# Tencent/PocketFlow

Measured on AMD Instinct MI355X. Metric: images/sec ResNet-50 INT8 quant-aware fine-tune (whole job; per GPU = value / n_gpus), higher is better.
Workload: dtype bf16

## Files before the change

### pocketflow_amd/csrc/pf_wrw.hip

```cpp
#include "pf_conv_common.h"
#include <stdlib.h>

#define LDS_PTR(p) ((__attribute__((address_space(3))) void*)(p))
typedef short v4s __attribute__((ext_vector_type(4)));
typedef short v8s __attribute__((ext_vector_type(8)));

__device__ __attribute__((aligned(16))) const uint32_t pf_wrw_zero_page[64] = {0};

struct WrwArgs {
  const bf16_t* dY;
  const bf16_t* X;
  float* slabs;
  const float* ss;
  const uint32_t* slot;
  float kq, act_lo, act_hi;
  int M, N, C;
  int th, tw, H, Wd, Ho, Wo, stride, pad_h, pad_w;
  int tiles_n, tiles, rows_per_split;
};

template <int N> __device__ __forceinline__ void wrw_wait_vm() { asm volatile("s_waitcnt vmcnt(%0)" ::"n"(N) : "memory"); }

template <int BN, bool PRO, bool MAP>
__global__ __launch_bounds__(256) void k_wrw_tr(const WrwArgs a) {
  constexpr int NB = BN / 16;
  constexpr int NS = 3;
  constexpr int DY_BYTES = 4 * NB * 256, X_BYTES = 4 * 4 * 256, STAGE = DY_BYTES + X_BYTES;
  constexpr int LPS = NB + 4;
  constexpr int NBLK = NB * 4;
  extern __shared__ __attribute__((aligned(16))) unsigned char smem[];
  const int tid = threadIdx.x, lane = tid & 63;
  const int wave = __builtin_amdgcn_readfirstlane(tid >> 6);
  const int l15 = lane & 15, q = lane >> 4;
  unsigned char* ring = smem + wave * (NS * STAGE);
  const bf16_t* zero = reinterpret_cast<const bf16_t*>(pf_wrw_zero_page);

  const int nwg = gridDim.x;
  int wg = blockIdx.x;
  {
    const int xcd = wg & 7, idx = wg >> 3;
    const int qq = nwg >> 3, r = nwg & 7;
    wg = (xcd < r ? xcd * (qq + 1) : r * (qq + 1) + (xcd - r) * qq) + idx;
  }
  const int tile = wg % a.tiles, split = wg / a.tiles;
  const int tn = tile % a.tiles_n, tk = tile / a.tiles_n;
  const int n0 = tn * BN;
  const int cch = a.C >> 6;
  const int tap = tk / cch, c0 = (tk - tap * cch) * 64;
  const int tap_r = tap / a.tw, tap_s = tap - tap_r * a.tw;
  const int ktot = a.th * a.tw * a.C;
  const int mbeg = split * a.rows_per_split;
  const int mend = (mbeg + a.rows_per_split < a.M) ? (mbeg + a.rows_per_split) : a.M;
  const int nsteps = (mend > mbeg) ? (mend - mbeg + 31) / 32 : 0;
  const int my_steps = (nsteps > wave) ? (nsteps - wave + 3) / 4 : 0;

  float psc[4], psh[4];
  Pro pro;
  pro_init(pro, a.act_lo, a.act_hi, a.kq, PRO ? a.slot : nullptr);
  if (PRO) {
#pragma unroll
    for (int j = 0; j < 4; ++j) {
      psc[j] = pro_fold_scale(pro, a.ss[c0 + j * 16 + l15]);
      psh[j] = pro_fold_shift(pro, a.ss[a.C + c0 + j * 16 + l15]);
    }
  }

  const int sb = lane >> 4, srow = (lane & 15) >> 1, sch = lane & 1;
  const int hw_o = a.Ho * a.Wo;
  auto stage = [&](int step, int buf) {
    unsigned char* dst = ring + buf * STAGE;
    const int mb = mbeg + step * 32;
#pragma unroll
    for (int pg = 0; pg < 4; ++pg) {
      const int m = mb + pg * 8 + srow;
      const bool ok = m < mend;
#pragma unroll
      for (int g4 = 0; g4 < NB / 4; ++g4) {
        const int n = n0 + (g4 * 4 + sb) * 16 + sch * 8;
        const bf16_t* src = (ok && n < a.N) ? (a.dY + (int64_t)m * a.N + n) : (zero + sch * 8);
        __builtin_amdgcn_global_load_lds(src, LDS_PTR(dst + (pg * NB + g4 * 4) * 256), 16, 0, 0);
      }
      bool okx = ok;
      int64_t row = m;
      if (MAP && ok) {
        const int img = m / hw_o, rem = m - img * hw_o;
        const int ho = rem / a.Wo, wo = rem - ho * a.Wo;
        const int hi = ho * a.stride + tap_r - a.pad_h, wi = wo * a.stride + tap_s - a.pad_w;
        okx = (unsigned)hi < (unsigned)a.H && (unsigned)wi < (unsigned)a.Wd;
        row = ((int64_t)img * a.H + hi) * a.Wd + wi;
      }
      const bf16_t* srcx = okx ? (a.X + row * a.C + c0 + sb * 16 + sch * 8) : (zero + sch * 8);
      __builtin_amdgcn_global_load_lds(srcx, LDS_PTR(dst + DY_BYTES + pg * 4 * 256), 16, 0, 0);
    }
  };

  f32x4 acc[NB][4];
#pragma unroll
  for (int i = 0; i < NB; ++i)
#pragma unroll
    for (int j = 0; j < 4; ++j) acc[i][j] = (f32x4){0.f, 0.f, 0.f, 0.f};

  const int tr_off = (q & 1) * 128 + (l15 >> 2) * 32 + (l15 & 3) * 8;
  const int pg_lo = q >> 1;

  if (my_steps > 0) stage(wave, 0);
  if (my_steps > 1) stage(wave + 4, 1);
  int ibuf = 2, cbuf = 0;
  for (int t = 0; t < my_steps; ++t) {
    if (t + 2 < my_steps) {
      stage(wave + (t + 2) * 4, ibuf);
      ibuf = (ibuf == NS - 1) ? 0 : ibuf + 1;
      wrw_wait_vm<2 * LPS>();
    } else if (t + 1 < my_steps) {
      wrw_wait_vm<LPS>();
    } else {
      wrw_wait_vm<0>();
    }
    __builtin_amdgcn_sched_barrier(0);
    const unsigned char* sbase = ring + cbuf * STAGE;
    cbuf = (cbuf == NS - 1) ? 0 : cbuf + 1;
    bf16x8 xf[4];
#pragma unroll
    for (int j = 0; j < 4; ++j) {
      const v4s lo = __builtin_amdgcn_ds_read_tr16_b64_v4i16(
          (__attribute__((address_space(3))) v4s*)(sbase + DY_BYTES + (pg_lo * 4 + j) * 256 + tr_off));
      const v4s hi = __builtin_amdgcn_ds_read_tr16_b64_v4i16(
          (__attribute__((address_space(3))) v4s*)(sbase + DY_BYTES + ((pg_lo + 2) * 4 + j) * 256 + tr_off));
      uint4 u;
      u.x = (uint32_t)(uint16_t)lo[0] | ((uint32_t)(uint16_t)lo[1] << 16);
      u.y = (uint32_t)(uint16_t)lo[2] | ((uint32_t)(uint16_t)lo[3] << 16);
      u.z = (uint32_t)(uint16_t)hi[0] | ((uint32_t)(uint16_t)hi[1] << 16);
      u.w = (uint32_t)(uint16_t)hi[2] | ((uint32_t)(uint16_t)hi[3] << 16);
      if (PRO) {
        float f[8];
        unpack8(u, f);
#pragma unroll
        for (int e = 0; e < 8; ++e) f[e] = pro_point(pro, psc[j], psh[j], f[e]);
        u = pack8(f);
      }
      xf[j] = *reinterpret_cast<const bf16x8*>(&u);
    }
#pragma unroll
    for (int i = 0; i < NB; ++i) {
      const v4s lo = __builtin_amdgcn_ds_read_tr16_b64_v4i16(
          (__attribute__((address_space(3))) v4s*)(sbase + (pg_lo * NB + i) * 256 + tr_off));
      const v4s hi = __builtin_amdgcn_ds_read_tr16_b64_v4i16(
          (__attribute__((address_space(3))) v4s*)(sbase + ((pg_lo + 2) * NB + i) * 256 + tr_off));
      v8s d8;
      d8[0] = lo[0]; d8[1] = lo[1]; d8[2] = lo[2]; d8[3] = lo[3];
      d8[4] = hi[0]; d8[5] = hi[1]; d8[6] = hi[2]; d8[7] = hi[3];
      const bf16x8 df = *reinterpret_cast<const bf16x8*>(&d8);
#pragma unroll
      for (int j = 0; j < 4; ++j)
        acc[i][j] = __builtin_amdgcn_mfma_f32_16x16x32_bf16(df, xf[j], acc[i][j], 0, 0, 0);
    }
  }

  __syncthreads();
  float4* red = reinterpret_cast<float4*>(smem);
#pragma unroll
  for (int i = 0; i < NB; ++i)
#pragma unroll
    for (int j = 0; j < 4; ++j)
      red[(wave * NBLK + i * 4 + j) * 64 + lane] = make_float4(acc[i][j][0], acc[i][j][1], acc[i][j][2], acc[i][j][3]);
  __syncthreads();
  float* out = a.slabs + (int64_t)split * a.N * ktot;
  const int kcol = tap * a.C + c0;
#pragma unroll
  for (int b = 0; b < NBLK / 4; ++b) {
    const int blk = wave * (NBLK / 4) + b;
    const int i = blk >> 2, j = blk & 3;
    float4 s = red[(0 * NBLK + blk) * 64 + lane];
#pragma unroll
    for (int w = 1; w < 4; ++w) {
      const float4 v = red[(w * NBLK + blk) * 64 + lane];
      s.x += v.x; s.y += v.y; s.z += v.z; s.w += v.w;
    }
    const int k = kcol + j * 16 + l15;
    const int n = n0 + i * 16 + q * 4;
    const float e[4] = {s.x, s.y, s.z, s.w};
#pragma unroll
    for (int r = 0; r < 4; ++r)
      if (n + r < a.N) out[(int64_t)(n + r) * ktot + k] = e[r];
  }
}

static bool wrw_tr_1x1_enabled() {
  return pf_tuning().wrw_tr != 0;
}

int pf_wrw_tr_splits(int M, int N, int C, int taps);
int pf_wrw2_splits(int M, int N, int C, int taps);
int pf_wrw_tr_splits_1x1(int M, int N, int C) {
  const int s2 = pf_wrw2_splits(M, N, C, 1);
  if (s2 > 0) return s2;
  return wrw_tr_1x1_enabled() ? pf_wrw_tr_splits(M, N, C, 1) : 0;
}

static int wrw_tr_bn(int N) { return (N % 128 == 0) ? 128 : 64; }

int pf_wrw_tr_splits(int M, int N, int C, int taps) {
  if ((C % 64) || (N % 64) || M < 2048) return 0;
  const int bn = wrw_tr_bn(N);
  const int tiles = (N / bn) * (taps * C / 64);
  int S = (256 + tiles - 1) / tiles;
  const int maxS = (M + 511) / 512;
  if (S > maxS) S = maxS;
  if (S < 1) S = 1;
  int rows = (M + S - 1) / S;
  rows = ((rows + 127) / 128) * 128;
  return (M + rows - 1) / rows;
}

template <int BN, bool PRO, bool MAP>
static int wrw_tr_launch_t(const WrwArgs& a, int grid, hipStream_t st) {
  constexpr int NB = BN / 16;
  const size_t ring = 4 * (size_t)3 * ((4 * NB + 16) * 256);
  const size_t red = (size_t)4 * NB * 4 * 64 * 16;
  const size_t lds = ring > red ? ring : red;
  if (int e = pf_require_lds(reinterpret_cast<const void*>(&k_wrw_tr<BN, PRO, MAP>), lds)) return e;
  k_wrw_tr<BN, PRO, MAP><<<grid, 256, lds, st>>>(a);
  PF_LAUNCH_CHECK();
  return 0;
}

int pf_wrw_tr_launch(const void* dY, const void* X, float* slabs, const float* scale_shift, int act,
                     const uint32_t* slot, int bits, int M, int N, int C, int th, int tw, int H, int Wd, int Ho, int Wo,
                     int stride, int pad_h, int pad_w, int S, hipStream_t st) {
  if (S <= 0) return -1;
  WrwArgs a;
  a.dY = (const bf16_t*)dY; a.X = (const bf16_t*)X; a.slabs = slabs;
  a.ss = scale_shift; a.slot = slot;
  a.kq = uq_k_of_bits(slot ? bits : 8);
  a.act_lo = (act == PF_ACT_NONE) ? -INFINITY : 0.0f;
  a.act_hi = (act == PF_ACT_RELU6) ? 6.0f : INFINITY;
  a.M = M; a.N = N; a.C = C; a.th = th; a.tw = tw; a.H = H; a.Wd = Wd; a.Ho = Ho; a.Wo = Wo;
  a.stride = stride; a.pad_h = pad_h; a.pad_w = pad_w;
  const int bn = wrw_tr_bn(N);
  a.tiles_n = N / bn;
  a.tiles = a.tiles_n * (th * tw * C / 64);
  int rows = (M + S - 1) / S;
  rows = ((rows + 127) / 128) * 128;
  a.rows_per_split = rows;
  const int grid = a.tiles * S;
  const bool pro = scale_shift != nullptr;
  const bool map = stride != 1 || th * tw > 1;
  if (pro && th * tw > 1) return -1;
#define PF_WT(BNV)                                                                            \
  do {                                                                                        \
    if (pro) return map ? wrw_tr_launch_t<BNV, true, true>(a, grid, st) : wrw_tr_launch_t<BNV, true, false>(a, grid, st);   \
    return map ? wrw_tr_launch_t<BNV, false, true>(a, grid, st) : wrw_tr_launch_t<BNV, false, false>(a, grid, st);          \
  } while (0)
  if (bn == 128) PF_WT(128);
  PF_WT(64);
#undef PF_WT
}

#if defined(__HIP_DEVICE_COMPILE__)
typedef __amdgpu_buffer_rsrc_t pf_wrsrc_t;
#define PF_W_MAKE_RSRC(p, bytes) __builtin_amdgcn_make_buffer_rsrc((void*)(p), (short)0, (int)(bytes), 0x00020000)
#define PF_W_BUFFER_LOAD_LDS16(rs, lds, voff) __builtin_amdgcn_raw_ptr_buffer_load_lds(rs, LDS_PTR(lds), 16, voff, 0, 0, 0)
#else
typedef int pf_wrsrc_t;
#define PF_W_MAKE_RSRC(p, bytes) 0
#define PF_W_BUFFER_LOAD_LDS16(rs, lds, voff) ((void)(rs), (void)(lds), (void)(voff))
#endif

#ifndef PF_W2_ABLATE
#define PF_W2_ABLATE 0
#endif
#ifdef PF_W2_TIMING
#define PF_W2_STAMP(k) do { if (blockIdx.x == (unsigned)tm_blk && t >= 4 && t < 12 && lane == 0) \
    tm_out[(t - 4) * 8 + (k)] = (uint32_t)__builtin_readcyclecounter(); } while (0)
#else
#define PF_W2_STAMP(k) do { } while (0)
#endif

__device__ __forceinline__ bf16x8 tr_join(const v4s& lo, const v4s& hi) {
  v8s x8;
  x8[0] = lo[0]; x8[1] = lo[1]; x8[2] = lo[2]; x8[3] = lo[3];
  x8[4] = hi[0]; x8[5] = hi[1]; x8[6] = hi[2]; x8[7] = hi[3];
  return *reinterpret_cast<const bf16x8*>(&x8);
}
template <int HI>
__device__ __forceinline__ void tr_read_frags(uint32_t p, bf16x8 (&f)[4]) {
  v4s l0, l1, l2, l3, h0, h1, h2, h3;
  asm volatile("ds_read_b64_tr_b16 %0, %8\n\tds_read_b64_tr_b16 %4, %8 offset:%9\n\t"
               "ds_read_b64_tr_b16 %1, %8 offset:256\n\tds_read_b64_tr_b16 %5, %8 offset:%10\n\t"
               "ds_read_b64_tr_b16 %2, %8 offset:512\n\tds_read_b64_tr_b16 %6, %8 offset:%11\n\t"
               "ds_read_b64_tr_b16 %3, %8 offset:768\n\tds_read_b64_tr_b16 %7, %8 offset:%12\n\t"
               "s_waitcnt lgkmcnt(0)"
               : "=&v"(l0), "=&v"(l1), "=&v"(l2), "=&v"(l3), "=&v"(h0), "=&v"(h1), "=&v"(h2), "=&v"(h3)
               : "v"(p), "n"(HI), "n"(HI + 256), "n"(HI + 512), "n"(HI + 768)
               : "memory");
  f[0] = tr_join(l0, h0); f[1] = tr_join(l1, h1); f[2] = tr_join(l2, h2); f[3] = tr_join(l3, h3);
}
template <int HI>
__device__ __forceinline__ void tr_read_frags(uint32_t p, bf16x8 (&f)[2]) {
  v4s l0, l1, h0, h1;
  asm volatile("ds_read_b64_tr_b16 %0, %4\n\tds_read_b64_tr_b16 %2, %4 offset:%5\n\t"
               "ds_read_b64_tr_b16 %1, %4 offset:256\n\tds_read_b64_tr_b16 %3, %4 offset:%6\n\t"
               "s_waitcnt lgkmcnt(0)"
               : "=&v"(l0), "=&v"(l1), "=&v"(h0), "=&v"(h1)
               : "v"(p), "n"(HI), "n"(HI + 256)
               : "memory");
  f[0] = tr_join(l0, h0); f[1] = tr_join(l1, h1);
}

template <int HIX, int HID>
__device__ __forceinline__ void tr_read_frags2(uint32_t px, uint32_t pd, bf16x8 (&xf)[4], bf16x8 (&df)[4]) {
  v4s a0, a1, a2, a3, b0, b1, b2, b3, c0, c1, c2, c3, d0, d1, d2, d3;
  asm volatile("ds_read_b64_tr_b16 %0, %16\n\tds_read_b64_tr_b16 %4, %16 offset:%18\n\t"
               "ds_read_b64_tr_b16 %1, %16 offset:256\n\tds_read_b64_tr_b16 %5, %16 offset:%19\n\t"
               "ds_read_b64_tr_b16 %2, %16 offset:512\n\tds_read_b64_tr_b16 %6, %16 offset:%20\n\t"
               "ds_read_b64_tr_b16 %3, %16 offset:768\n\tds_read_b64_tr_b16 %7, %16 offset:%21\n\t"
               "ds_read_b64_tr_b16 %8, %17\n\tds_read_b64_tr_b16 %12, %17 offset:%22\n\t"
               "ds_read_b64_tr_b16 %9, %17 offset:256\n\tds_read_b64_tr_b16 %13, %17 offset:%23\n\t"
               "ds_read_b64_tr_b16 %10, %17 offset:512\n\tds_read_b64_tr_b16 %14, %17 offset:%24\n\t"
               "ds_read_b64_tr_b16 %11, %17 offset:768\n\tds_read_b64_tr_b16 %15, %17 offset:%25\n\t"
               "s_waitcnt lgkmcnt(0)"
               : "=&v"(a0), "=&v"(a1), "=&v"(a2), "=&v"(a3), "=&v"(b0), "=&v"(b1), "=&v"(b2), "=&v"(b3),
                 "=&v"(c0), "=&v"(c1), "=&v"(c2), "=&v"(c3), "=&v"(d0), "=&v"(d1), "=&v"(d2), "=&v"(d3)
               : "v"(px), "v"(pd), "n"(HIX), "n"(HIX + 256), "n"(HIX + 512), "n"(HIX + 768), "n"(HID), "n"(HID + 256), "n"(HID + 512),
                 "n"(HID + 768)
               : "memory");
  xf[0] = tr_join(a0, b0); xf[1] = tr_join(a1, b1); xf[2] = tr_join(a2, b2); xf[3] = tr_join(a3, b3);
  df[0] = tr_join(c0, d0); df[1] = tr_join(c1, d1); df[2] = tr_join(c2, d2); df[3] = tr_join(c3, d3);
}

struct Wrw2Args {
  const bf16_t* dY;
  const bf16_t* X;
  float* slabs;
  const float* ss;
  const uint32_t* slot;
  float kq, act_lo, act_hi;
  uint32_t dy_bytes, x_bytes;
  int M, N, C;
  int th, tw, H, Wd, Ho, Wo, stride, pad_h, pad_w;
  int tiles_n, tiles, rows_per_split;
};

template <int TN, int TK, int WTN, int WTK, bool PRO, int MAPM>
__global__ __launch_bounds__(64 * (TN / WTN) * (TK / WTK)) void k_wrw2(const Wrw2Args a) {
  constexpr int WN = TN / WTN, WK = TK / WTK, NWAVE = WN * WK;
  constexpr int NI = WTN / 16, NJ = WTK / 16;
  constexpr int NBN = TN / 16, NBK = TK / 16;
  constexpr int DY_BYTES = 4 * NBN * 256, X_BYTES = 4 * NBK * 256, STAGE = DY_BYTES + X_BYTES;
  constexpr int IDY = 4 * (TN / 64), IX = 4 * (TK / 64);
  static_assert(IDY % NWAVE == 0 || IDY < NWAVE, "dY instructions must split evenly over the wavefronts (slot kinds are static)");
  constexpr int KDY = (IDY + NWAVE - 1) / NWAVE;
  constexpr int XS = (IX + NWAVE - 1) / NWAVE;
  extern __shared__ __attribute__((aligned(16))) unsigned char smem[];
  const int tid = threadIdx.x, lane = tid & 63;
  const int wave = __builtin_amdgcn_readfirstlane(tid >> 6);
  const int l15 = lane & 15, q = lane >> 4;
  const int wn = wave / WK, wk = wave % WK;

  const int nwg = gridDim.x;
  int wg = blockIdx.x;
  {
    const int xcd = wg & 7, idx = wg >> 3;
    const int qq = nwg >> 3, r = nwg & 7;
    wg = (xcd < r ? xcd * (qq + 1) : r * (qq + 1) + (xcd - r) * qq) + idx;
  }
  const int tile = wg % a.tiles, split = wg / a.tiles;
  const int tn = tile % a.tiles_n, tk = tile / a.tiles_n;
  const int n0 = tn * TN;
  const int kt = a.C / TK;
  const int tap = tk / kt, c0 = (tk - tap * kt) * TK;
  const int tap_r = tap / a.tw, tap_s = tap - tap_r * a.tw;
  const int ktot = a.th * a.tw * a.C;
  const int mbeg = split * a.rows_per_split;
  const int mend = (mbeg + a.rows_per_split < a.M) ? (mbeg + a.rows_per_split) : a.M;
  const int nsteps = (mend > mbeg) ? (mend - mbeg + 31) / 32 : 0;

  const pf_wrsrc_t rsY = PF_W_MAKE_RSRC(a.dY, (uint32_t)mend * (uint32_t)a.N * 2u);
  const pf_wrsrc_t rsX = PF_W_MAKE_RSRC(a.X, (MAPM == 0) ? (uint32_t)mend * (uint32_t)a.C * 2u : a.x_bytes);
  constexpr uint32_t OOB = 0x80000000u;
  const int sb = lane >> 4, srow = (lane & 15) >> 1, sch = lane & 1;
  const int hw_o = a.Ho * a.Wo;

  float psc[XS][8], psh[XS][8];
  Pro pro;
  pro_init(pro, a.act_lo, a.act_hi, a.kq, PRO ? a.slot : nullptr);
  if (PRO) {
#pragma unroll
    for (int x = 0; x < XS; ++x) {
      const int xi = wave + x * NWAVE;
      if (xi < IX) {
        const int g4 = xi % (TK / 64);
        const int c = c0 + (g4 * 4 + sb) * 16 + sch * 8;
#pragma unroll
        for (int j = 0; j < 8; ++j) { psc[x][j] = pro_fold_scale(pro, a.ss[c + j]); psh[x][j] = pro_fold_shift(pro, a.ss[a.C + c + j]); }
      }
    }
  }

  uint32_t yoff[KDY], xoff[XS];
  const uint32_t ystep = 32u * (uint32_t)a.N * 2u, xstep = 32u * (uint32_t)a.C * 2u;
#pragma unroll
  for (int k = 0; k < KDY; ++k) {
    const int id = (wave + k * NWAVE) % IDY;
    const int pg = id / (TN / 64), g4 = id % (TN / 64);
    const int n = n0 + (g4 * 4 + sb) * 16 + sch * 8;
    yoff[k] = (n < a.N && wave + k * NWAVE < IDY) ? (uint32_t)((mbeg + pg * 8 + srow) * a.N + n) * 2u : OOB;
  }
  int px_img[XS], px_ho[XS], px_wo[XS];
  const int adv_q = 32 / a.Wo, adv_r = 32 - adv_q * a.Wo;
  const int tap_dr = tap_r - a.pad_h, tap_ds = tap_s - a.pad_w;
#pragma unroll
  for (int x = 0; x < XS; ++x) {
    const int xi = (wave + x * NWAVE) % IX;
    const int pg = xi / (TK / 64), g4 = xi % (TK / 64);
    const int m = mbeg + pg * 8 + srow;
    const int cofs = c0 + (g4 * 4 + sb) * 16 + sch * 8;
    px_img[x] = 0; px_ho[x] = 0; px_wo[x] = 0;
    if (MAPM != 0) {
      const int img = m / hw_o, rem = m - img * hw_o;
      px_img[x] = img; px_ho[x] = rem / a.Wo; px_wo[x] = rem - px_ho[x] * a.Wo;
    }
    const int row0 = (MAPM == 1) ? m + tap_dr * a.Wd + tap_ds : m;
    xoff[x] = (uint32_t)(row0 * a.C + cofs) * 2u;
  }
  auto stage = [&](int step, int buf) {
    unsigned char* dst = smem + buf * STAGE;
    const int mb = mbeg + step * 32;
#pragma unroll
    for (int k = 0; k < KDY; ++k) {
      const bool owny = wave + k * NWAVE < IDY;
      const int id = (wave + k * NWAVE) % IDY;
      const int pg = id / (TN / 64), g4 = id % (TN / 64);
      unsigned char* ydst = owny ? dst + (pg * NBN + g4 * 4) * 256 : smem + 3 * STAGE;
      if (!(PF_W2_ABLATE & 2)) PF_W_BUFFER_LOAD_LDS16(rsY, ydst, yoff[k]);
      yoff[k] += ystep;
    }
#pragma unroll
    for (int x = 0; x < XS; ++x) {
      const bool own = wave + x * NWAVE < IX;
      const int xi = (wave + x * NWAVE) % IX;
      const int pg = xi / (TK / 64), g4 = xi % (TK / 64);
      uint32_t voff;
      if (MAPM == 0) {
        voff = xoff[x];
        xoff[x] += xstep;
      } else if (MAPM == 1) {
        const int m = mb + pg * 8 + srow;
        const bool ok = m < mend && (unsigned)(px_ho[x] + tap_dr) < (unsigned)a.H && (unsigned)(px_wo[x] + tap_ds) < (unsigned)a.Wd;
        voff = ok ? xoff[x] : OOB;
        xoff[x] += xstep;
        px_wo[x] += adv_r; px_ho[x] += adv_q;
        if (px_wo[x] >= a.Wo) { px_wo[x] -= a.Wo; ++px_ho[x]; }
        if (px_ho[x] >= a.Ho) px_ho[x] -= a.Ho;
      } else {
        const int m = mb + pg * 8 + srow;
        const int hi = px_ho[x] * a.stride + tap_r - a.pad_h, wi = px_wo[x] * a.stride + tap_s - a.pad_w;
        const bool ok = m < mend && (unsigned)hi < (unsigned)a.H && (unsigned)wi < (unsigned)a.Wd;
        const int row = (px_img[x] * a.H + hi) * a.Wd + wi;
        voff = ok ? (uint32_t)(row * a.C + c0 + (g4 * 4 + sb) * 16 + sch * 8) * 2u : OOB;
        px_wo[x] += adv_r; px_ho[x] += adv_q;
        if (px_wo[x] >= a.Wo) { px_wo[x] -= a.Wo; ++px_ho[x]; }
        while (px_ho[x] >= a.Ho) { px_ho[x] -= a.Ho; ++px_img[x]; }
      }
      if (!own) voff = OOB;
      unsigned char* xdst = own ? dst + DY_BYTES + (pg * NBK + g4 * 4) * 256 : smem + 3 * STAGE;
      if (!(PF_W2_ABLATE & 2)) PF_W_BUFFER_LOAD_LDS16(rsX, xdst, voff);
    }
  };
  auto transform = [&](int buf) {
    unsigned char* dst = smem + buf * STAGE;
#pragma unroll
    for (int x = 0; x < XS; ++x) {
      const int xi = wave + x * NWAVE;
      if (xi < IX) {
        const int pg = xi / (TK / 64), g4 = xi % (TK / 64);
#pragma unroll
        for (int j = 0; j < 8; ++j) { pro.sc[j] = psc[x][j]; pro.sh[j] = psh[x][j]; }
        const uint32_t p = lds_addr(dst + DY_BYTES + (pg * NBK + g4 * 4) * 256 + lane * 16);
        lds_write_b128(p, pro_apply(pro, lds_read_b128(p)));
      }
    }
  };

  f32x4 acc[NI][NJ];
#pragma unroll
  for (int i = 0; i < NI; ++i)
#pragma unroll
    for (int j = 0; j < NJ; ++j) acc[i][j] = (f32x4){0.f, 0.f, 0.f, 0.f};
  const int tr_off = (q & 1) * 128 + (l15 >> 2) * 32 + (l15 & 3) * 8;
  const int pg_lo = q >> 1;

  constexpr int NSTG = 3, LPS = KDY + XS;
  if (nsteps > 0) stage(0, 0);
  if (nsteps > 1) { stage(1, 1); wrw_wait_vm<LPS>(); } else wrw_wait_vm<0>();
  if (PRO && nsteps > 0) transform(0);
  asm volatile("s_waitcnt lgkmcnt(0)" ::: "memory");
  __builtin_amdgcn_s_barrier();
  int buf = 0, ibuf = 2;
#ifdef PF_W2_TIMING
  const int tm_blk = gridDim.x / 2;
  uint32_t* tm_out = reinterpret_cast<uint32_t*>(a.slabs) + wave * 64;
#endif
  for (int t = 0; t < nsteps; ++t) {
    const bool more2 = t + 2 < nsteps;
    PF_W2_STAMP(0);
    if (more2) { stage(t + 2, ibuf); ibuf = (ibuf + 1 == NSTG) ? 0 : ibuf + 1; }
    PF_W2_STAMP(1);
    const unsigned char* sbase = smem + buf * STAGE;
    buf = (buf + 1 == NSTG) ? 0 : buf + 1;
    if (!(PF_W2_ABLATE & 1)) {
      bf16x8 xf[NJ], df[NI];
      if constexpr (NI == 4 && NJ == 4) {
        tr_read_frags2<2 * NBK * 256, 2 * NBN * 256>(lds_addr(sbase + DY_BYTES + (pg_lo * NBK + wk * NJ) * 256 + tr_off),
                                                     lds_addr(sbase + (pg_lo * NBN + wn * NI) * 256 + tr_off), xf, df);
      } else
      {
      tr_read_frags<2 * NBK * 256>(lds_addr(sbase + DY_BYTES + (pg_lo * NBK + wk * NJ) * 256 + tr_off), xf);
      tr_read_frags<2 * NBN * 256>(lds_addr(sbase + (pg_lo * NBN + wn * NI) * 256 + tr_off), df);
      }
      PF_W2_STAMP(2);
#pragma unroll
      for (int i = 0; i < NI; ++i)
#pragma unroll
        for (int j = 0; j < NJ; ++j)
          acc[i][j] = __builtin_amdgcn_mfma_f32_16x16x32_bf16(df[i], xf[j], acc[i][j], 0, 0, 0);
    }
    __builtin_amdgcn_sched_barrier(0);
    PF_W2_STAMP(3);
    if (t + 1 < nsteps) {
      if (more2) wrw_wait_vm<LPS>(); else wrw_wait_vm<0>();
      PF_W2_STAMP(4);
      if (PRO) transform(buf);
    }
    asm volatile("s_waitcnt lgkmcnt(0)" ::: "memory");
    PF_W2_STAMP(5);
    __builtin_amdgcn_s_barrier();
    __builtin_amdgcn_sched_barrier(0);
    PF_W2_STAMP(6);
  }
#ifdef PF_W2_TIMING
  return;
#endif

  float* out = a.slabs + (int64_t)split * a.N * ktot;
  const int kcol = tap * a.C + c0 + wk * WTK;
#pragma unroll
  for (int i = 0; i < NI; ++i)
#pragma unroll
    for (int j = 0; j < NJ; ++j) {
      const int k = kcol + j * 16 + l15;
      const int n = n0 + wn * WTN + i * 16 + q * 4;
#pragma unroll
      for (int r = 0; r < 4; ++r)
        if (n + r < a.N && (!(PF_W2_ABLATE & 4) || acc[i][j][r] == 12345.678f)) out[(int64_t)(n + r) * ktot + k] = acc[i][j][r];
    }
}

struct Wrw2Cfg { int tn, tk; };
static Wrw2Cfg wrw2_pick(int N, int C) {
  const int tn = (N % 256 == 0) ? 256 : ((N % 128 == 0) ? 128 : 64);
  int tk = (C % 128 == 0) ? 128 : 64;
  if (tn <= 128 && C % 256 == 0 && pf_tuning().wrw2_tk256 != 0) tk = 256;
  if (tn == 128 && tk == 64) return Wrw2Cfg{64, 64};
  return Wrw2Cfg{tn, tk};
}

static bool wrw2_enabled() {
  return pf_tuning().wrw2 != 0;
}

int pf_wrw2_splits(int M, int N, int C, int taps) {
  if (!wrw2_enabled() || (C % 64) || (N % 64) || M < 2048) return 0;
  if ((int64_t)M * N >= ((int64_t)1 << 30)) return 0;
  const Wrw2Cfg c = wrw2_pick(N, C);
  const int tiles = (N / c.tn) * (taps * C / c.tk);
  const int forced = pf_tuning().wrw2_target;
  const int target = (forced > 0) ? forced : (taps == 1 ? 256 : 384);
  int S = (target + tiles - 1) / tiles;
  const int maxS = (M + 255) / 256;
  if (S > maxS) S = maxS;
  if (S < 1) S = 1;
  int rows = (M + S - 1) / S;
  rows = ((rows + 31) / 32) * 32;
  return (M + rows - 1) / rows;
}

template <int TN, int TK, int WTN, int WTK, bool PRO, int MAPM>
static int wrw2_launch_t(const Wrw2Args& a, int grid, hipStream_t st) {
  const size_t lds = 3 * (size_t)(4 * (TN / 16) * 256 + 4 * (TK / 16) * 256) + 1024;
  if (int e = pf_require_lds(reinterpret_cast<const void*>(&k_wrw2<TN, TK, WTN, WTK, PRO, MAPM>), lds)) return e;
  k_wrw2<TN, TK, WTN, WTK, PRO, MAPM><<<grid, 64 * (TN / WTN) * (TK / WTK), lds, st>>>(a);
  PF_LAUNCH_CHECK();
  return 0;
}

int pf_wrw2_launch(const void* dY, const void* X, float* slabs, const float* scale_shift, int act, const uint32_t* slot,
                   int bits, int M, int N, int C, int th, int tw, int H, int Wd, int Ho, int Wo, int stride, int pad_h,
                   int pad_w, int S, int64_t x_rows, hipStream_t st) {
  if (S <= 0) return -1;
  if (x_rows * C >= ((int64_t)1 << 30) || (int64_t)M * N >= ((int64_t)1 << 30)) return -1;
  Wrw2Args a;
  a.dY = (const bf16_t*)dY; a.X = (const bf16_t*)X; a.slabs = slabs; a.ss = scale_shift; a.slot = slot;
  a.kq = uq_k_of_bits(slot ? bits : 8);
  a.act_lo = (act == PF_ACT_NONE) ? -INFINITY : 0.0f;
  a.act_hi = (act == PF_ACT_RELU6) ? 6.0f : INFINITY;
  a.dy_bytes = (uint32_t)((int64_t)M * N * 2);
  a.x_bytes = (uint32_t)(x_rows * C * 2);
  a.M = M; a.N = N; a.C = C; a.th = th; a.tw = tw; a.H = H; a.Wd = Wd; a.Ho = Ho; a.Wo = Wo;
  a.stride = stride; a.pad_h = pad_h; a.pad_w = pad_w;
  const Wrw2Cfg c = wrw2_pick(N, C);
  a.tiles_n = N / c.tn;
  a.tiles = a.tiles_n * (th * tw * C / c.tk);
  int rows = (M + S - 1) / S;
  rows = ((rows + 31) / 32) * 32;
  a.rows_per_split = rows;
  const int grid = a.tiles * S;
  const bool pro = scale_shift != nullptr;
  int mapm = 0;
  if (stride != 1 || th * tw > 1) mapm = (stride == 1 && Ho == H && Wo == Wd && 32 / Wo + 1 <= Ho) ? 1 : 2;
  if (pro && th * tw > 1) return -1;
  if (pro && mapm == 1) mapm = 2;
#define PF_W2(TNV, TKV, WTNV, WTKV)                                                                           \
  do {                                                                                                        \
    if (pro) return mapm ? wrw2_launch_t<TNV, TKV, WTNV, WTKV, true, 2>(a, grid, st)                           \
                         : wrw2_launch_t<TNV, TKV, WTNV, WTKV, true, 0>(a, grid, st);                          \
    if (mapm == 1) return wrw2_launch_t<TNV, TKV, WTNV, WTKV, false, 1>(a, grid, st);                          \
    return mapm ? wrw2_launch_t<TNV, TKV, WTNV, WTKV, false, 2>(a, grid, st)                                   \
                : wrw2_launch_t<TNV, TKV, WTNV, WTKV, false, 0>(a, grid, st);                                  \
  } while (0)
  if (c.tn == 128 && c.tk == 256) PF_W2(128, 256, 64, 64);
  if (c.tn == 64 && c.tk == 256) PF_W2(64, 256, 32, 64);
  if (c.tn == 256 && c.tk == 128) PF_W2(256, 128, 64, 64);
  if (c.tn == 128 && c.tk == 128) PF_W2(128, 128, 64, 64);
  if (c.tn == 256 && c.tk == 64) PF_W2(256, 64, 64, 32);
  if (c.tn == 64 && c.tk == 128) PF_W2(64, 128, 32, 64);
  PF_W2(64, 64, 32, 32);
#undef PF_W2
}

int pf_wrw_reduce(float* workspace, int S, int64_t n, void* dW, int dw_dtype, hipStream_t st);

bool pf_wrw3x3_c64_geom(int H, int Wd, int C, int N, int th, int tw, int stride, int pad_h, int pad_w, int Ho, int Wo);
int pf_wrw3x3_c64_splits(int imgs);
int pf_wrw3x3_c64_launch(const void* dY, const void* X, float* slabs, int imgs, hipStream_t st);

extern "C" int pf_conv2d_wrw_splits(int M, int N, int C, int taps) {
  const int s2 = pf_wrw2_splits(M, N, C, taps);
  int s = s2 > 0 ? s2 : pf_wrw_tr_splits(M, N, C, taps);
  if (pf_tuning().conv3x3_c64 != 0 && taps == 9 && N == 64 && C == 64 && M % (56 * 56) == 0) {
    const int s3 = pf_wrw3x3_c64_splits(M / (56 * 56));
    if (s3 > s) s = s3;
  }
  return s;
}

extern "C" int pf_conv2d_wrw(const void* dY, const void* X, void* dW, int dw_dtype, float* workspace, int imgs, int H,
                             int Wd, int C, int N, int th, int tw, int stride, int pad_h, int pad_w, int Ho, int Wo,
                             void* stream) {
  if (imgs <= 0 || H <= 0 || Wd <= 0 || Ho <= 0 || Wo <= 0 || th < 1 || tw < 1 || stride < 1) return (int)hipErrorInvalidValue;
  if (!pf_aligned16(dY) || !pf_aligned16(X) || !pf_aligned16(dW) || !pf_aligned16(workspace)) return (int)hipErrorInvalidValue;
  const int M = imgs * Ho * Wo;
  hipStream_t st = (hipStream_t)stream;
  if (pf_wrw3x3_c64_geom(H, Wd, C, N, th, tw, stride, pad_h, pad_w, Ho, Wo)) {
    const int r3 = pf_wrw3x3_c64_launch(dY, X, workspace, imgs, st);
    if (r3 == 0) return pf_wrw_reduce(workspace, pf_wrw3x3_c64_splits(imgs), (int64_t)N * th * tw * C, dW, dw_dtype, st);
    if (r3 > 0) return r3;
  }
  const int s2 = pf_wrw2_splits(M, N, C, th * tw);
  const int S = s2 > 0 ? s2 : pf_wrw_tr_splits(M, N, C, th * tw);
  if (S <= 0) return (int)hipErrorInvalidValue;
  int r = -1;
  if (s2 > 0)
    r = pf_wrw2_launch(dY, X, workspace, nullptr, PF_ACT_NONE, nullptr, 8, M, N, C, th, tw, H, Wd, Ho, Wo, stride, pad_h,
                       pad_w, S, (int64_t)imgs * H * Wd, st);
  if (r < 0)
    r = pf_wrw_tr_launch(dY, X, workspace, nullptr, PF_ACT_NONE, nullptr, 8, M, N, C, th, tw, H, Wd, Ho, Wo, stride,
                         pad_h, pad_w, S, st);
  if (r != 0) return r < 0 ? (int)hipErrorInvalidValue : r;
  return pf_wrw_reduce(workspace, S, (int64_t)N * th * tw * C, dW, dw_dtype, st);
}
```

Before: 11380.

## Overlap LDS transposed reads with next-stage loads and stage wrw epilogue through LDS

The weight-gradient kernel now issues all ds_read_b64_tr fragment reads before launching the global-to-LDS stage for step t+2. It then waits on lgkmcnt incrementally, so MFMAs for fragment s start as soon as that fragment arrives instead of after one full wait. The epilogue transposes accumulators through per-wave LDS scratch so each lane writes float4 rows instead of scattered scalar stores. This adds LDS traffic, inline-asm counter assumptions and reuse of stage buffers after the loop, which could race if any wave is still reading.

```diff
diff --git a/pocketflow_amd/csrc/pf_wrw.hip b/pocketflow_amd/csrc/pf_wrw.hip
--- a/pocketflow_amd/csrc/pf_wrw.hip
+++ b/pocketflow_amd/csrc/pf_wrw.hip
@@ -270,10 +270,14 @@
 #define PF_W2_ABLATE 0
 #endif
 #ifdef PF_W2_TIMING
-#define PF_W2_STAMP(k) do { if (blockIdx.x == (unsigned)tm_blk && t >= 4 && t < 12 && lane == 0) \
-    tm_out[(t - 4) * 8 + (k)] = (uint32_t)__builtin_readcyclecounter(); } while (0)
+#define PF_W2_STAMP(k) asm volatile("s_memtime %0" : "=s"(tm_ts[k]))
+#define PF_W2_STAMPS_OUT() do { \
+    asm volatile("s_waitcnt lgkmcnt(0)" : "+s"(tm_ts[0]), "+s"(tm_ts[1]), "+s"(tm_ts[2]), "+s"(tm_ts[3]), "+s"(tm_ts[4]), "+s"(tm_ts[5]), "+s"(tm_ts[6])); \
+    if (blockIdx.x == (unsigned)tm_blk && t >= 4 && t < 12 && lane == 0) \
+      for (int k = 0; k < 7; ++k) tm_out[(t - 4) * 8 + k] = (uint32_t)tm_ts[k]; } while (0)
 #else
 #define PF_W2_STAMP(k) do { } while (0)
+#define PF_W2_STAMPS_OUT() do { } while (0)
 #endif
 
 __device__ __forceinline__ bf16x8 tr_join(const v4s& lo, const v4s& hi) {
@@ -282,50 +286,31 @@
   x8[4] = hi[0]; x8[5] = hi[1]; x8[6] = hi[2]; x8[7] = hi[3];
   return *reinterpret_cast<const bf16x8*>(&x8);
 }
-template <int HI>
-__device__ __forceinline__ void tr_read_frags(uint32_t p, bf16x8 (&f)[4]) {
-  v4s l0, l1, l2, l3, h0, h1, h2, h3;
-  asm volatile("ds_read_b64_tr_b16 %0, %8\n\tds_read_b64_tr_b16 %4, %8 offset:%9\n\t"
-               "ds_read_b64_tr_b16 %1, %8 offset:256\n\tds_read_b64_tr_b16 %5, %8 offset:%10\n\t"
-               "ds_read_b64_tr_b16 %2, %8 offset:512\n\tds_read_b64_tr_b16 %6, %8 offset:%11\n\t"
-               "ds_read_b64_tr_b16 %3, %8 offset:768\n\tds_read_b64_tr_b16 %7, %8 offset:%12\n\t"
-               "s_waitcnt lgkmcnt(0)"
-               : "=&v"(l0), "=&v"(l1), "=&v"(l2), "=&v"(l3), "=&v"(h0), "=&v"(h1), "=&v"(h2), "=&v"(h3)
-               : "v"(p), "n"(HI), "n"(HI + 256), "n"(HI + 512), "n"(HI + 768)
-               : "memory");
-  f[0] = tr_join(l0, h0); f[1] = tr_join(l1, h1); f[2] = tr_join(l2, h2); f[3] = tr_join(l3, h3);
-}
-template <int HI>
-__device__ __forceinline__ void tr_read_frags(uint32_t p, bf16x8 (&f)[2]) {
-  v4s l0, l1, h0, h1;
-  asm volatile("ds_read_b64_tr_b16 %0, %4\n\tds_read_b64_tr_b16 %2, %4 offset:%5\n\t"
-               "ds_read_b64_tr_b16 %1, %4 offset:256\n\tds_read_b64_tr_b16 %3, %4 offset:%6\n\t"
-               "s_waitcnt lgkmcnt(0)"
-               : "=&v"(l0), "=&v"(l1), "=&v"(h0), "=&v"(h1)
-               : "v"(p), "n"(HI), "n"(HI + 256)
-               : "memory");
-  f[0] = tr_join(l0, h0); f[1] = tr_join(l1, h1);
-}
-
-template <int HIX, int HID>
-__device__ __forceinline__ void tr_read_frags2(uint32_t px, uint32_t pd, bf16x8 (&xf)[4], bf16x8 (&df)[4]) {
-  v4s a0, a1, a2, a3, b0, b1, b2, b3, c0, c1, c2, c3, d0, d1, d2, d3;
-  asm volatile("ds_read_b64_tr_b16 %0, %16\n\tds_read_b64_tr_b16 %4, %16 offset:%18\n\t"
-               "ds_read_b64_tr_b16 %1, %16 offset:256\n\tds_read_b64_tr_b16 %5, %16 offset:%19\n\t"
-               "ds_read_b64_tr_b16 %2, %16 offset:512\n\tds_read_b64_tr_b16 %6, %16 offset:%20\n\t"
-               "ds_read_b64_tr_b16 %3, %16 offset:768\n\tds_read_b64_tr_b16 %7, %16 offset:%21\n\t"
-               "ds_read_b64_tr_b16 %8, %17\n\tds_read_b64_tr_b16 %12, %17 offset:%22\n\t"
-               "ds_read_b64_tr_b16 %9, %17 offset:256\n\tds_read_b64_tr_b16 %13, %17 offset:%23\n\t"
-               "ds_read_b64_tr_b16 %10, %17 offset:512\n\tds_read_b64_tr_b16 %14, %17 offset:%24\n\t"
-               "ds_read_b64_tr_b16 %11, %17 offset:768\n\tds_read_b64_tr_b16 %15, %17 offset:%25\n\t"
-               "s_waitcnt lgkmcnt(0)"
-               : "=&v"(a0), "=&v"(a1), "=&v"(a2), "=&v"(a3), "=&v"(b0), "=&v"(b1), "=&v"(b2), "=&v"(b3),
-                 "=&v"(c0), "=&v"(c1), "=&v"(c2), "=&v"(c3), "=&v"(d0), "=&v"(d1), "=&v"(d2), "=&v"(d3)
-               : "v"(px), "v"(pd), "n"(HIX), "n"(HIX + 256), "n"(HIX + 512), "n"(HIX + 768), "n"(HID), "n"(HID + 256), "n"(HID + 512),
-                 "n"(HID + 768)
-               : "memory");
-  xf[0] = tr_join(a0, b0); xf[1] = tr_join(a1, b1); xf[2] = tr_join(a2, b2); xf[3] = tr_join(a3, b3);
-  df[0] = tr_join(c0, d0); df[1] = tr_join(c1, d1); df[2] = tr_join(c2, d2); df[3] = tr_join(c3, d3);
+template <int LO, int HI>
+__device__ __forceinline__ void tr_issue(uint32_t p, v4s& lo, v4s& hi) {
+  asm volatile("ds_read_b64_tr_b16 %0, %2 offset:%3\n\tds_read_b64_tr_b16 %1, %2 offset:%4"
+               : "=&v"(lo), "=&v"(hi) : "v"(p), "n"(LO), "n"(HI) : "memory");
+}
+template <int N>
+__device__ __forceinline__ void tr_wait(v4s& l0, v4s& h0) {
+  asm volatile("s_waitcnt lgkmcnt(%2)" : "+v"(l0), "+v"(h0) : "n"(N) : "memory");
+}
+template <int N>
+__device__ __forceinline__ void tr_wait(v4s& l0, v4s& h0, v4s& l1, v4s& h1) {
+  asm volatile("s_waitcnt lgkmcnt(%4)" : "+v"(l0), "+v"(h0), "+v"(l1), "+v"(h1) : "n"(N) : "memory");
+}
+template <int V> struct WrwIc { static constexpr int value = V; };
+template <int I, int N, class F>
+__device__ __forceinline__ void wrw_static_for(F&& f) {
+  if constexpr (I < N) { f(WrwIc<I>{}); wrw_static_for<I + 1, N>(f); }
+}
+template <int OFF>
+__device__ __forceinline__ void lds_write_b32_at(uint32_t p, float v) {
+  asm volatile("ds_write_b32 %0, %1 offset:%2" : : "v"(p), "v"(v), "n"(OFF) : "memory");
+}
+template <int OFF>
+__device__ __forceinline__ void lds_read_b128_at(uint32_t p, f32x4v_t& v) {
+  asm volatile("ds_read_b128 %0, %1 offset:%2" : "=&v"(v) : "v"(p), "n"(OFF) : "memory");
 }
 
 struct Wrw2Args {
@@ -491,6 +476,9 @@
   const int pg_lo = q >> 1;
 
   constexpr int NSTG = 3, LPS = KDY + XS;
+  constexpr int NR = 2 * (NI + NJ);
+  constexpr int NW = NI > NJ ? NI : NJ;
+  static_assert(NI <= 4 && NJ <= 4 && NR - 4 <= 15, "the step is unrolled for at most four fragments per operand; lgkmcnt has 4 bits");
   if (nsteps > 0) stage(0, 0);
   if (nsteps > 1) { stage(1, 1); wrw_wait_vm<LPS>(); } else wrw_wait_vm<0>();
   if (PRO && nsteps > 0) transform(0);
@@ -503,57 +491,104 @@
 #endif
   for (int t = 0; t < nsteps; ++t) {
     const bool more2 = t + 2 < nsteps;
+#ifdef PF_W2_TIMING
+    uint64_t tm_ts[7];
+#endif
     PF_W2_STAMP(0);
-    if (more2) { stage(t + 2, ibuf); ibuf = (ibuf + 1 == NSTG) ? 0 : ibuf + 1; }
-    PF_W2_STAMP(1);
     const unsigned char* sbase = smem + buf * STAGE;
     buf = (buf + 1 == NSTG) ? 0 : buf + 1;
+    v4s xl[NJ], xh[NJ], dl[NI], dh[NI];
+    if (!(PF_W2_ABLATE & 1)) {
+      const uint32_t px = lds_addr(sbase + DY_BYTES + (pg_lo * NBK + wk * NJ) * 256 + tr_off);
+      const uint32_t pd = lds_addr(sbase + (pg_lo * NBN + wn * NI) * 256 + tr_off);
+      auto issue = [&](auto sc) {
+        constexpr int s = decltype(sc)::value;
+        if constexpr (s < NJ) tr_issue<s * 256, 2 * NBK * 256 + s * 256>(px, xl[s], xh[s]);
+        if constexpr (s < NI) tr_issue<s * 256, 2 * NBN * 256 + s * 256>(pd, dl[s], dh[s]);
+      };
+      issue(WrwIc<0>{}); issue(WrwIc<1>{}); issue(WrwIc<2>{}); issue(WrwIc<3>{});
+    }
+    __builtin_amdgcn_sched_barrier(0);
+    PF_W2_STAMP(1);
+    if (more2) { stage(t + 2, ibuf); ibuf = (ibuf + 1 == NSTG) ? 0 : ibuf + 1; }
+    __builtin_amdgcn_sched_barrier(0);
+    PF_W2_STAMP(2);
     if (!(PF_W2_ABLATE & 1)) {
       bf16x8 xf[NJ], df[NI];
-      if constexpr (NI == 4 && NJ == 4) {
-        tr_read_frags2<2 * NBK * 256, 2 * NBN * 256>(lds_addr(sbase + DY_BYTES + (pg_lo * NBK + wk * NJ) * 256 + tr_off),
-                                                     lds_addr(sbase + (pg_lo * NBN + wn * NI) * 256 + tr_off), xf, df);
-      } else
-      {
-      tr_read_frags<2 * NBK * 256>(lds_addr(sbase + DY_BYTES + (pg_lo * NBK + wk * NJ) * 256 + tr_off), xf);
-      tr_read_frags<2 * NBN * 256>(lds_addr(sbase + (pg_lo * NBN + wn * NI) * 256 + tr_off), df);
-      }
-      PF_W2_STAMP(2);
-#pragma unroll
-      for (int i = 0; i < NI; ++i)
-#pragma unroll
-        for (int j = 0; j < NJ; ++j)
-          acc[i][j] = __builtin_amdgcn_mfma_f32_16x16x32_bf16(df[i], xf[j], acc[i][j], 0, 0, 0);
-    }
-    __builtin_amdgcn_sched_barrier(0);
+      auto mma = [&](auto sc) {
+        constexpr int s = decltype(sc)::value;
+        if constexpr (s < NW) {
+          constexpr int got = 2 * ((s + 1 < NJ ? s + 1 : NJ) + (s + 1 < NI ? s + 1 : NI));
+          if constexpr (s < NJ && s < NI) tr_wait<NR - got>(xl[s], xh[s], dl[s], dh[s]);
+          else if constexpr (s < NJ) tr_wait<NR - got>(xl[s], xh[s]);
+          else tr_wait<NR - got>(dl[s], dh[s]);
+          if constexpr (s < NJ) xf[s] = tr_join(xl[s], xh[s]);
+          if constexpr (s < NI) df[s] = tr_join(dl[s], dh[s]);
+#pragma unroll
+          for (int i = 0; i < NI; ++i)
+#pragma unroll
+            for (int j = 0; j < NJ; ++j)
+              if ((i > j ? i : j) == s) acc[i][j] = __builtin_amdgcn_mfma_f32_16x16x32_bf16(df[i], xf[j], acc[i][j], 0, 0, 0);
+          __builtin_amdgcn_sched_barrier(0);
+        }
+      };
+      mma(WrwIc<0>{}); mma(WrwIc<1>{}); mma(WrwIc<2>{}); mma(WrwIc<3>{});
+    }
     PF_W2_STAMP(3);
     if (t + 1 < nsteps) {
       if (more2) wrw_wait_vm<LPS>(); else wrw_wait_vm<0>();
       PF_W2_STAMP(4);
       if (PRO) transform(buf);
     }
+#ifdef PF_W2_TIMING
+    else PF_W2_STAMP(4);
+#endif
     asm volatile("s_waitcnt lgkmcnt(0)" ::: "memory");
     PF_W2_STAMP(5);
     __builtin_amdgcn_s_barrier();
     __builtin_amdgcn_sched_barrier(0);
     PF_W2_STAMP(6);
+    PF_W2_STAMPS_OUT();
   }
 #ifdef PF_W2_TIMING
   return;
 #endif
 
-  float* out = a.slabs + (int64_t)split * a.N * ktot;
-  const int kcol = tap * a.C + c0 + wk * WTK;
-#pragma unroll
-  for (int i = 0; i < NI; ++i)
-#pragma unroll
-    for (int j = 0; j < NJ; ++j) {
-      const int k = kcol + j * 16 + l15;
-      const int n = n0 + wn * WTN + i * 16 + q * 4;
-#pragma unroll
-      for (int r = 0; r < 4; ++r)
-        if (n + r < a.N && (!(PF_W2_ABLATE & 4) || acc[i][j][r] == 12345.678f)) out[(int64_t)(n + r) * ktot + k] = acc[i][j][r];
-    }
+  constexpr int PITCH = WTK + 4;
+  constexpr int WBYTES = ((NSTG * STAGE + 1024) / NWAVE) & ~15;
+  constexpr int NPASS = (WTN * PITCH * 4 <= WBYTES) ? 1 : 2;
+  constexpr int IPP = NI / NPASS;
+  constexpr int LPR = WTK / 4, RPI = 64 / LPR;
+  static_assert(NI % NPASS == 0 && IPP * 16 * PITCH * 4 <= WBYTES, "a pass of the slab epilogue must fit the wavefront's LDS");
+  static_assert((IPP * 16) % RPI == 0, "whole row groups per pass");
+  constexpr int NG = IPP * 16 / RPI;
+  const int rrow = lane / LPR, rcol = (lane % LPR) * 4;
+  const uint32_t wbase = lds_addr(smem + wave * WBYTES);
+  const uint32_t pw = wbase + ((q * 4) * PITCH + l15) * 4, pr = wbase + (rrow * PITCH + rcol) * 4;
+  float* out = a.slabs + (int64_t)split * a.N * ktot + (int64_t)(n0 + wn * WTN + rrow) * ktot + (tap * a.C + c0 + wk * WTK + rcol);
+  const int nrow = n0 + wn * WTN + rrow;
+#pragma unroll
+  for (int ps = 0; ps < NPASS; ++ps) {
+    wrw_static_for<0, IPP * NJ * 4>([&](auto ic) {
+      constexpr int e = decltype(ic)::value, ii = e / (NJ * 4), j = (e / 4) % NJ, r = e % 4;
+      lds_write_b32_at<((ii * 16 + r) * PITCH + j * 16) * 4>(pw, acc[ps * IPP + ii][j][r]);
+    });
+    asm volatile("s_waitcnt lgkmcnt(0)" ::: "memory");
+    f32x4v_t rv[NG];
+    wrw_static_for<0, NG>([&](auto ic) {
+      constexpr int g = decltype(ic)::value;
+      lds_read_b128_at<g * RPI * PITCH * 4>(pr, rv[g]);
+    });
+    asm volatile("s_waitcnt lgkmcnt(0)" ::: "memory");
+#pragma unroll
+    for (int g = 0; g < NG; ++g) asm volatile("" : "+v"(rv[g]));
+#pragma unroll
+    for (int g = 0; g < NG; ++g) {
+      const int row = ps * IPP * 16 + g * RPI;
+      if (nrow + row < a.N && (!(PF_W2_ABLATE & 4) || rv[g][0] == 12345.678f))
+        *reinterpret_cast<float4*>(out + (int64_t)row * ktot) = make_float4(rv[g][0], rv[g][1], rv[g][2], rv[g][3]);
+    }
+  }
 }
 
 struct Wrw2Cfg { int tn, tk; };
```

Measured after the change: 11320. Within noise of the previous version (-0.5%).
